# ibrahimhroob/SPS

Hardware: AMD Instinct MI355X
Metric: scans/sec @100k pts, 0.1 m voxel (higher is better)
Workload: dtype f32; 1 GPU; BASELINE config 2: single ~100k-pt LiDAR-like scan + variant-B submap, 0.1 m voxel, CustomMinkUNet14 fp32, 1 scan per step per GPU (4 distinct scans cycled); scan_points=100824, rows=153557, streams_per_gpu=8, compact_arenas=True

## Files before the change

### sps_amd/csrc/grid_kernels.inc.h

```cpp

typedef unsigned int u32x2 __attribute__((ext_vector_type(2)));
constexpr int SCAN_BLOCK = 1024;

struct BHash {
  uint64_t *keys;
  unsigned long long *mask;
  int *first;
  int *rank;
  uint32_t *occ;
  uint32_t hmask;
  uint32_t hshift;
};

constexpr uint32_t BH_X = 0x9E3779B1u, BH_Y = 0x85EBCA77u, BH_Z = 0xC2B2AE3Du, BH_T = 0x27D4EB2Fu;
__device__ inline uint32_t bhash32(uint64_t key) {
  return (uint32_t)(key & 0x3FFFF) * BH_X + (uint32_t)((key >> 18) & 0x3FFFF) * BH_Y + (uint32_t)((key >> 36) & 0x3FFFF) * BH_Z +
         (uint32_t)(key >> 54) * BH_T;
}

__device__ inline int bhash_insert(const BHash &h, uint64_t key) {
  uint32_t s = bhash32(key) >> h.hshift;
  while (true) {
    unsigned long long prev = atomicCAS(reinterpret_cast<unsigned long long *>(&h.keys[s]),
                                        (unsigned long long)KEY_EMPTY, (unsigned long long)key);
    if (prev == KEY_EMPTY) atomicOr(&h.occ[s >> 5], 1u << (s & 31));
    if (prev == KEY_EMPTY || prev == key) return (int)s;
    s = (s + 1) & h.hmask;
  }
}
__device__ inline int bhash_find_from(const BHash &h, uint64_t key, uint32_t s) {
  while (true) {
    if (!((h.occ[s >> 5] >> (s & 31)) & 1u)) return -1;
    if (h.keys[s] == key) return (int)s;
    s = (s + 1) & h.hmask;
  }
}
__device__ inline int bhash_find(const BHash &h, uint64_t key) {
  uint32_t s = bhash32(key) >> h.hshift;
  while (true) {
    if (!((h.occ[s >> 5] >> (s & 31)) & 1u)) return -1;
    if (h.keys[s] == key) return (int)s;
    s = (s + 1) & h.hmask;
  }
}

__device__ inline uint64_t bkey_pack(uint32_t b, uint32_t tt, uint32_t bx, uint32_t by, uint32_t bz) {
  return ((uint64_t)b << 59) | ((uint64_t)tt << 54) | ((uint64_t)bz << 36) | ((uint64_t)by << 18) | (uint64_t)bx;
}

constexpr int NLV = SPS_NUM_LEVELS;

__device__ inline int wave_run_insert(const BHash &h, uint64_t key, bool ok, uint32_t olo, uint32_t ohi, int src) {
  const int lane = threadIdx.x & 63;
  const uint32_t klo = (uint32_t)key, khi = (uint32_t)(key >> 32);
  const uint32_t plo = __shfl_up(klo, 1, 64), phi = __shfl_up(khi, 1, 64);
  const int pok = __shfl_up((int)ok, 1, 64);
  const bool head = !(lane > 0 && ok && pok && plo == klo && phi == khi);
  const unsigned long long heads = __ballot(head);
  const unsigned long long le = heads & (lane == 63 ? ~0ull : ((2ull << lane) - 1ull));
  const int rid = __popcll(le);
  const int head_lane = 63 - __clzll((long long)le);
  if (!ok) {
    olo = 0u;
    ohi = 0u;
  }
#pragma unroll
  for (int o = 1; o < 64; o <<= 1) {
    const uint32_t vlo = __shfl_down(olo, o, 64), vhi = __shfl_down(ohi, o, 64);
    const int r2 = __shfl_down(rid, o, 64);
    if (lane + o < 64 && r2 == rid) {
      olo |= vlo;
      ohi |= vhi;
    }
  }
  int slot = -1;
  if (head && ok) {
    if constexpr (SPS_ABLATE_FE & 1) {
      slot = (int)(bhash32(key) >> h.hshift);
    } else {
      slot = bhash_insert(h, key);
      atomicOr(&h.mask[slot], ((unsigned long long)ohi << 32) | olo);
      atomicMin(&h.first[slot], src);
    }
  }
  return __shfl(slot, head_lane, 64);
}

__global__ __launch_bounds__(256) void k_points_to_blocks(const float *__restrict__ coords, int64_t ld, int n, float vs,
                                                           float t_base, BHash h, int *__restrict__ sslot,
                                                           unsigned char *__restrict__ sbit, int *err,
                                                           uint4 *__restrict__ zero_region, int zero_vec4,
                                                           double *__restrict__ metrics_zero, int metrics_n,
                                                           const int *__restrict__ n_dev) {
  if (n_dev) n = min(n, *n_dev);
  const int p = blockIdx.x * blockDim.x + threadIdx.x;
  if (p < metrics_n) metrics_zero[p] = 0.0;
  for (int i = p; i < zero_vec4; i += gridDim.x * blockDim.x) zero_region[i] = make_uint4(0u, 0u, 0u, 0u);
  bool ok = false;
  uint64_t key = KEY_EMPTY;
  int bit = 0;
  if (p < n) {
    const float *c = coords + (size_t)p * ld;
    const float fb = floorf(__fdiv_rn(c[0], 1.0f));
    const float fx = floorf(__fdiv_rn(c[1], vs));
    const float fy = floorf(__fdiv_rn(c[2], vs));
    const float fz = floorf(__fdiv_rn(c[3], vs));
    const float ft = floorf(__fdiv_rn(c[4], 1.0f)) - t_base;
    ok = fb >= 0.f && fb <= (float)SPS_BATCH_MAX && ft >= (float)SPS_T_MIN && ft <= (float)SPS_T_MAX &&
         fx >= (float)SPS_COORD_MIN && fx <= (float)SPS_COORD_MAX && fy >= (float)SPS_COORD_MIN &&
         fy <= (float)SPS_COORD_MAX && fz >= (float)SPS_COORD_MIN && fz <= (float)SPS_COORD_MAX;
    if (ok) {
      const uint32_t ux = (uint32_t)((int)fx + XBIAS), uy = (uint32_t)((int)fy + XBIAS), uz = (uint32_t)((int)fz + XBIAS);
      key = bkey_pack((uint32_t)(int)fb, (uint32_t)((int)ft + TBIAS), ux >> 2, uy >> 2, uz >> 2);
      bit = (int)(((uz & 3) << 4) | ((uy & 3) << 2) | (ux & 3));
    } else {
      atomicOr(err, 1);
    }
  }
  const int slot = wave_run_insert(h, key, ok, bit < 32 ? (1u << bit) : 0u, bit >= 32 ? (1u << (bit - 32)) : 0u, p);
  if (p < n) {
    sslot[p] = ok ? slot : -1;
    sbit[p] = (unsigned char)bit;
  }
}

struct PyramidArgs {
  BHash h[NLV];
  int *sslot[NLV];
  const unsigned char *sbit0;
  int *bslot[NLV];
  uint64_t *bkey[NLV];
  unsigned long long *bmask[NLV];
  int *bbase[NLV];
  uint4 *bmb[NLV];
  int *bparent[NLV];
  int *bchild[NLV];
  int *badj[NLV];
  int *vblock[NLV];
  unsigned char *vbit[NLV];
  int *counts;
  unsigned long long *agg;
  int agg_stride;
  uint32_t gen;
  const int *n_dev;
  int capl[NLV], bcapl[NLV];
  int *err;
};

constexpr int ABORT = 15;

__device__ inline int block_reduce_sum(int v, int *lds) {
  const int lane = threadIdx.x & 63, wave = threadIdx.x >> 6;
  for (int o = 32; o > 0; o >>= 1) v += __shfl_down(v, o, 64);
  if (lane == 0) lds[wave] = v;
  __syncthreads();
  int tot = 0;
  const int nw = blockDim.x >> 6;
  for (int i = 0; i < nw; ++i) tot += lds[i];
  __syncthreads();
  return tot;
}

constexpr int TICKET = 16, TOCC = 24, N_COUNTERS = 32;

__device__ inline unsigned long long agg_pack(uint32_t gen, int t0, int t1) {
  return ((unsigned long long)gen << 32) | ((unsigned long long)(uint32_t)t1 << 13) | (unsigned long long)(uint32_t)t0;
}
constexpr int SCAN_SPIN_MAX = 1 << 22;
__device__ inline int2 scan_lookback(const unsigned long long *agg, int id, uint32_t gen, int *lds, int *err) {
  if constexpr (SPS_ABLATE_FE & 2) return make_int2(0, 0);
  int p0 = 0, p1 = 0;
  for (int i = threadIdx.x; i < id; i += SCAN_BLOCK) {
    unsigned long long v = __hip_atomic_load(agg + i, __ATOMIC_RELAXED, __HIP_MEMORY_SCOPE_AGENT);
    for (int spin = 0; (uint32_t)(v >> 32) != gen; ++spin) {
      if (spin == SCAN_SPIN_MAX) {
        atomicOr(err, 16);
        v = 0ull;
        break;
      }
      __builtin_amdgcn_s_sleep(1);
      v = __hip_atomic_load(agg + i, __ATOMIC_RELAXED, __HIP_MEMORY_SCOPE_AGENT);
    }
    p0 += (int)(v & 0x1FFFull);
    p1 += (int)((v >> 13) & 0x7FFFFull);
  }
  const int b0 = block_reduce_sum(p0, lds);
  const int b1 = block_reduce_sum(p1, lds);
  return make_int2(b0, b1);
}
__device__ inline int2 block_exclusive_scan2(int v0, int v1, int2 *wave_off, int2 &tot) {
  const int lane = threadIdx.x & 63, wave = threadIdx.x >> 6;
  int i0 = v0, i1 = v1;
  for (int o = 1; o < 64; o <<= 1) {
    const int t0 = __shfl_up(i0, o, 64), t1 = __shfl_up(i1, o, 64);
    if (lane >= o) {
      i0 += t0;
      i1 += t1;
    }
  }
  if (lane == 63) wave_off[wave] = make_int2(i0, i1);
  __syncthreads();
  int o0 = 0, o1 = 0, s0 = 0, s1 = 0;
  for (int i = 0; i < SCAN_BLOCK / 64; ++i) {
    const int2 w = wave_off[i];
    if (i < wave) o0 += w.x, o1 += w.y;
    s0 += w.x, s1 += w.y;
  }
  __syncthreads();
  tot = make_int2(s0, s1);
  return make_int2(o0 + i0 - v0, o1 + i1 - v1);
}

#if defined(SPS_FE_TRACE)
__device__ unsigned long long g_fe_trace[8 * 4096];
#define FE_STAMP(kernel, k) do { if (threadIdx.x == 0) g_fe_trace[8 * ((kernel) * 1024 + blockIdx.x) + (k)] = wall_clock64(); } while (0)
#else
#define FE_STAMP(kernel, k) do { } while (0)
#endif
struct Ranked {
  int flag, slot, rank, base;
  unsigned long long mask;
  uint64_t key;
  int wg_rank0, wg_blocks;
};
template <int ITEMS>
__device__ inline bool rank_pass(const PyramidArgs &a, int l, int n, Ranked &o, int *lds, int2 *wave_off, int *sh_id) {
  FE_STAMP(l != 0, 0);
  if (threadIdx.x == 0) *sh_id = atomicAdd(&a.counts[TICKET + l], 1);
  __syncthreads();
  const int id = *sh_id;
  FE_STAMP(l != 0, 1);
  constexpr int PER_WG = SCAN_BLOCK * ITEMS;
  const int nwg = (n + PER_WG - 1) / PER_WG;
  if (id >= nwg) return false;
  const int p0 = id * PER_WG + (int)threadIdx.x * ITEMS;
  int s[ITEMS], cnt[ITEMS];
  unsigned long long m[ITEMS];
  int flags = 0, nf = 0, nv = 0;
  if (ITEMS == 4 && p0 + 3 < n) {
    const int4 v = *reinterpret_cast<const int4 *>(a.sslot[l] + p0);
    s[0] = v.x, s[1 % ITEMS] = v.y, s[2 % ITEMS] = v.z, s[3 % ITEMS] = v.w;
  } else {
#pragma unroll
    for (int i = 0; i < ITEMS; ++i) s[i] = p0 + i < n ? a.sslot[l][p0 + i] : -1;
  }
  int first[ITEMS];
  uint64_t key[ITEMS];
#pragma unroll
  for (int i = 0; i < ITEMS; ++i) {
    const int si = max(s[i], 0);
    first[i] = a.h[l].first[si];
    m[i] = a.h[l].mask[si];
    key[i] = a.h[l].keys[si];
  }
#pragma unroll
  for (int i = 0; i < ITEMS; ++i) {
    cnt[i] = 0;
    if (s[i] >= 0 && first[i] == p0 + i) {
      flags |= 1 << i;
      cnt[i] = __popcll(m[i]);
      ++nf, nv += cnt[i];
    }
  }
  int2 tot;
  const int2 loc = block_exclusive_scan2(nf, nv, wave_off, tot);
  unsigned long long *agg = a.agg + (size_t)l * a.agg_stride;
  if (threadIdx.x == 0) __hip_atomic_store(agg + id, agg_pack(a.gen, tot.x, tot.y), __ATOMIC_RELAXED, __HIP_MEMORY_SCOPE_AGENT);
  FE_STAMP(l != 0, 2);
  const int2 base = scan_lookback(agg, id, a.gen, lds, a.err);
  FE_STAMP(l != 0, 3);
  int r = base.x + loc.x, vb = base.y + loc.y;
  o.flag = 0;
  o.wg_rank0 = base.x, o.wg_blocks = tot.x;
#pragma unroll
  for (int i = 0; i < ITEMS; ++i) {
    if (((flags >> i) & 1) && r < a.bcapl[l]) {
      a.h[l].rank[s[i]] = r;
      a.bslot[l][r] = s[i];
      a.bkey[l][r] = key[i];
      a.bmask[l][r] = m[i];
      a.bbase[l][r] = vb;
      a.bmb[l][r] = make_uint4((uint32_t)m[i], (uint32_t)(m[i] >> 32), (uint32_t)vb, 0u);
      int4 *ch = reinterpret_cast<int4 *>(a.bchild[l] + (size_t)r * 8);
      ch[0] = make_int4(-1, -1, -1, -1);
      ch[1] = make_int4(-1, -1, -1, -1);
      if (ITEMS == 1) o.flag = 1, o.slot = s[i], o.rank = r, o.base = vb, o.mask = m[i], o.key = key[i];
    }
    if ((flags >> i) & 1) ++r, vb += cnt[i];
  }
  if (id == nwg - 1 && threadIdx.x == 0) {
    const int nb = base.x + tot.x, nvx = base.y + tot.y;
    a.counts[8 + l] = min(nb, a.bcapl[l]);
    a.counts[l] = nvx;
    if (nb > a.bcapl[l] || nvx > a.capl[l]) {
      atomicOr(&a.counts[ABORT], 1);
      atomicOr(a.err, 2);
    }
  }
  return true;
}

__global__ __launch_bounds__(SCAN_BLOCK) void k_rank_points(PyramidArgs a, int n0) {
  __shared__ int lds[SCAN_BLOCK / 64];
  __shared__ int2 wave_off[SCAN_BLOCK / 64];
  __shared__ int sh_id;
  __shared__ uint64_t sh_key[SCAN_BLOCK];
  __shared__ unsigned long long sh_mask[SCAN_BLOCK];
  const int n = a.n_dev ? min(n0, *a.n_dev) : n0;
  Ranked k;
  if (!rank_pass<1>(a, 0, n, k, lds, wave_off, &sh_id)) return;
  FE_STAMP(0, 4);
  uint32_t tb = 0u;
  if (k.flag) {
    const uint64_t key = k.key;
    sh_key[k.rank - k.wg_rank0] = key;
    sh_mask[k.rank - k.wg_rank0] = k.mask;
    tb = 1u << (uint32_t)((key >> 54) & 0x1F);
  }
  for (int o = 32; o > 0; o >>= 1) tb |= __shfl_xor(tb, o, 64);
  if ((threadIdx.x & 63) == 0) lds[threadIdx.x >> 6] = (int)tb;
  __syncthreads();
  if (threadIdx.x == 0) {
    for (int i = 1; i < SCAN_BLOCK / 64; ++i) tb |= (uint32_t)lds[i];
    uint32_t *tocc = reinterpret_cast<uint32_t *>(a.counts) + TOCC;
    if ((__hip_atomic_load(tocc, __ATOMIC_RELAXED, __HIP_MEMORY_SCOPE_AGENT) & tb) != tb) atomicOr(tocc, tb);
  }
  const int nb = min(k.wg_blocks, a.bcapl[0] - k.wg_rank0);
  const int lane = threadIdx.x & 63, wave = threadIdx.x >> 6;
  FE_STAMP(0, 5);
  const int l = 1 + (wave & 3);
  for (int j0 = (wave >> 2) * 64; j0 < nb; j0 += 256) {
    const int j = j0 + lane;
    const bool ok = j < nb;
    uint64_t pkey = KEY_EMPTY;
    unsigned long long pm = 0;
    if (ok) {
      const uint64_t key = sh_key[j];
      const uint32_t bx = (uint32_t)(key & 0x3FFFF), by = (uint32_t)((key >> 18) & 0x3FFFF), bz = (uint32_t)((key >> 36) & 0x3FFFF);
      const uint64_t bt = key & (0x3FFull << 54);
      pkey = bt | ((uint64_t)(bz >> l) << 36) | ((uint64_t)(by >> l) << 18) | (uint64_t)(bx >> l);
      if (l == 1) {
        const unsigned long long m = sh_mask[j];
        const uint32_t ox = bx & 1, oy = by & 1, oz = bz & 1;
#pragma unroll
        for (int kk = 0; kk < 2; ++kk)
#pragma unroll
          for (int jj = 0; jj < 2; ++jj)
#pragma unroll
            for (int i = 0; i < 2; ++i)
              if (m & (0x0000000000330033ull << (2 * i + 8 * jj + 32 * kk)))
                pm |= 1ull << ((2 * oz + kk) * 16 + (2 * oy + jj) * 4 + (2 * ox + i));
      } else {
        const uint32_t px = (bx >> (l - 2)) & 3, py = (by >> (l - 2)) & 3, pz = (bz >> (l - 2)) & 3;
        pm = 1ull << ((pz << 4) | (py << 2) | px);
      }
    }
    const int r = k.wg_rank0 + j;
    int sl = 0;
    if constexpr (!(SPS_ABLATE_FE & 4))
      sl = wave_run_insert(a.h[l], pkey, ok, (uint32_t)pm, (uint32_t)(pm >> 32), r);
    if (ok) a.sslot[l][r] = sl;
  }
#if defined(SPS_FE_TRACE)
  __syncthreads();
  FE_STAMP(0, 6);
#endif
}

constexpr int RANK_ITEMS = 1;
__global__ __launch_bounds__(SCAN_BLOCK) void k_rank_blocks_rows(PyramidArgs a, int gsb, int n0, int *__restrict__ inv) {
  __shared__ int lds[SCAN_BLOCK / 64];
  __shared__ int2 wave_off[SCAN_BLOCK / 64];
  __shared__ int sh_id;
  if ((int)blockIdx.x < 4 * gsb) {
    const int nblk = a.counts[8];
    if (((int)blockIdx.x % gsb) * (SCAN_BLOCK * RANK_ITEMS) >= nblk) return;
    Ranked k;
    rank_pass<RANK_ITEMS>(a, 1 + (int)blockIdx.x / gsb, nblk, k, lds, wave_off, &sh_id);
    FE_STAMP(1, 4);
    return;
  }
  if (a.counts[ABORT]) return;
  FE_STAMP(1, 0);
  const int n = a.n_dev ? min(n0, *a.n_dev) : n0;
  const int p = ((int)blockIdx.x - 4 * gsb) * SCAN_BLOCK + (int)threadIdx.x;
  if (p >= n) return;
  const int s = a.sslot[0][p];
  int row = -1;
  if (s >= 0) {
    const BHash &h = a.h[0];
    const int r = h.rank[s];
    const int bit = a.sbit0[p];
    row = a.bbase[0][r] + __popcll(h.mask[s] & ((1ull << bit) - 1ull));
    a.vblock[0][row] = r;
    a.vbit[0][row] = (unsigned char)bit;
  }
  inv[p] = row;
  FE_STAMP(1, 6);
}

__device__ inline void link_levels(const PyramidArgs &a, int l, int bx, int nbx) {
  const int n = a.counts[8 + l];
  for (int r = bx * 256 + (int)threadIdx.x; r < n; r += nbx * 256) {
    const uint64_t key = a.bkey[l][r];
    const uint32_t bx = (uint32_t)(key & 0x3FFFF), by = (uint32_t)((key >> 18) & 0x3FFFF),
                   bz = (uint32_t)((key >> 36) & 0x3FFFF);
    const uint64_t bt = key & (0x3FFull << 54);
    const uint64_t pkey = bt | ((uint64_t)(bz >> 1) << 36) | ((uint64_t)(by >> 1) << 18) | (uint64_t)(bx >> 1);
    const int ps = bhash_find(a.h[l + 1], pkey);
    const int pr = a.h[l + 1].rank[ps];
    a.bparent[l][r] = pr;
    a.bchild[l + 1][(size_t)pr * 8 + ((bx & 1) | ((by & 1) << 1) | ((bz & 1) << 2))] = r;
    if (l == 0) {
      const unsigned long long m = a.bmask[0][r];
      int sj[NLV], brj[NLV], basej[NLV];
      unsigned long long pmj[NLV];
#pragma unroll
      for (int j = 1; j < NLV; ++j) sj[j] = a.sslot[j][r];
#pragma unroll
      for (int j = 1; j < NLV; ++j) {
        brj[j] = a.h[j].rank[sj[j]];
        pmj[j] = a.h[j].mask[sj[j]];
      }
#pragma unroll
      for (int j = 1; j < NLV; ++j) basej[j] = a.bbase[j][brj[j]];
#pragma unroll
      for (int j = 1; j < NLV; ++j) {
        const int br = brj[j];
        const unsigned long long pmask = pmj[j];
        const int base = basej[j];
        if (j == 1) {
          const uint32_t ox = bx & 1, oy = by & 1, oz = bz & 1;
#pragma unroll
          for (int k = 0; k < 2; ++k)
#pragma unroll
            for (int jj = 0; jj < 2; ++jj)
#pragma unroll
              for (int i = 0; i < 2; ++i)
                if (m & (0x0000000000330033ull << (2 * i + 8 * jj + 32 * k))) {
                  const int bit = (int)((2 * oz + k) * 16 + (2 * oy + jj) * 4 + (2 * ox + i));
                  const int row = base + __popcll(pmask & ((1ull << bit) - 1ull));
                  a.vblock[1][row] = br;
                  a.vbit[1][row] = (unsigned char)bit;
                }
        } else {
          const uint32_t px = (bx >> (j - 2)) & 3, py = (by >> (j - 2)) & 3, pz = (bz >> (j - 2)) & 3;
          const int bit = (int)((pz << 4) | (py << 2) | px);
          const int row = base + __popcll(pmask & ((1ull << bit) - 1ull));
          a.vblock[j][row] = br;
          a.vbit[j][row] = (unsigned char)bit;
        }
      }
    }
  }
}

constexpr int LINK_PER = 3;
#if defined(SPS_FE_TRACE)
__device__ unsigned long long g_link_trace[2 * 16384];
struct LinkStamp {
  __device__ LinkStamp() { if (threadIdx.x == 0 && blockIdx.x < 16384) g_link_trace[2 * blockIdx.x] = wall_clock64(); }
  __device__ ~LinkStamp() { if (threadIdx.x == 0 && blockIdx.x < 16384) g_link_trace[2 * blockIdx.x + 1] = wall_clock64(); }
};
#endif
__global__ __launch_bounds__(256) void k_link_adj(PyramidArgs a, int gb, int c1, int c2, int c3, int c4, int c5) {
  if (a.counts[ABORT]) return;
#if defined(SPS_FE_TRACE)
  LinkStamp stamp;
#endif
  if ((int)blockIdx.x < 4 * gb) {
    link_levels(a, (int)blockIdx.x / gb, (int)blockIdx.x % gb, gb);
    return;
  }
  const int bx = (int)blockIdx.x - 4 * gb;
  const int idx = bx < c1 ? 0 : bx < c2 ? 1 : bx < c3 ? 2 : bx < c4 ? 3 : 4;
  const int level = NLV - 1 - idx;
  const int lo = idx == 0 ? 0 : idx == 1 ? c1 : idx == 2 ? c2 : idx == 3 ? c3 : c4;
  const int hi = idx == 0 ? c1 : idx == 1 ? c2 : idx == 2 ? c3 : idx == 3 ? c4 : c5;
  const int total = a.counts[8 + level] * 27;
  const int lim = 1 << (16 - level);
  const BHash h = a.h[level];
  const uint32_t tocc = reinterpret_cast<const uint32_t *>(a.counts)[TOCC];
  const uint64_t *__restrict__ bkey = a.bkey[level];
  int *__restrict__ badj = a.badj[level];
  const __amdgpu_buffer_rsrc_t rsOcc = __builtin_amdgcn_make_buffer_rsrc((void *)h.occ, 0, (int)0xFFFFFFFEu, 0x00020000);
  const __amdgpu_buffer_rsrc_t rsKeys = __builtin_amdgcn_make_buffer_rsrc((void *)h.keys, 0, (int)0xFFFFFFFEu, 0x00020000);
  const __amdgpu_buffer_rsrc_t rsRank = __builtin_amdgcn_make_buffer_rsrc((void *)h.rank, 0, (int)0xFFFFFFFEu, 0x00020000);
  for (int i = (bx - lo) * 256 + (int)threadIdx.x; i < total; i += (hi - lo) * 256) {
    const int r = i / 27, g = i - r * 27;
    const int dy = g % 3 - 1, dz = (g / 3) % 3 - 1, dt = g / 9 - 1;
    const uint64_t key = bkey[r];
    const int kx = (int)(key & 0x3FFFF), ky = (int)((key >> 18) & 0x3FFFF) + dy, kz = (int)((key >> 36) & 0x3FFFF) + dz,
              tt = (int)((key >> 54) & 0x1F) + dt;
    const bool gok = ky >= 0 && ky < lim && kz >= 0 && kz < lim && tt >= 0 && tt < 32 && ((tocc >> tt) & 1u);
    const uint64_t gkey = key + ((uint64_t)(int64_t)dy << 18) + ((uint64_t)(int64_t)dz << 36) + ((uint64_t)(int64_t)dt << 54);
    const uint32_t ghash = bhash32(key) + (uint32_t)dy * BH_Y + (uint32_t)dz * BH_Z + (uint32_t)dt * BH_T;
    uint64_t nk[LINK_PER];
    uint32_t sl[LINK_PER];
    int res[LINK_PER];
    bool probe[LINK_PER];
#pragma unroll
    for (int j = 0; j < LINK_PER; ++j) {
      const int dx = j - 1;
      const bool self = dx == 0 && g == 13;
      res[j] = self ? r : -1;
      probe[j] = !(SPS_ABLATE_FE & 8) && gok && !self && kx + dx >= 0 && kx + dx < lim;
      nk[j] = gkey + (uint64_t)(int64_t)dx;
      sl[j] = (ghash + (uint32_t)dx * BH_X) >> h.hshift;
    }
    uint32_t ow[LINK_PER];
#pragma unroll
    for (int j = 0; j < LINK_PER; ++j) ow[j] = __builtin_amdgcn_raw_buffer_load_b32(rsOcc, probe[j] ? (sl[j] >> 5) * 4u : 0xFFFFFFFFu, 0, 0);
    uint64_t k1[LINK_PER];
#pragma unroll
    for (int j = 0; j < LINK_PER; ++j) {
      probe[j] = probe[j] && ((ow[j] >> (sl[j] & 31)) & 1u);
      const u32x2 kv = __builtin_amdgcn_raw_buffer_load_b64(rsKeys, probe[j] ? sl[j] * 8u : 0xFFFFFFFFu, 0, 0);
      k1[j] = ((uint64_t)kv.y << 32) | kv.x;
    }
    bool hit[LINK_PER];
    int rk[LINK_PER];
#pragma unroll
    for (int j = 0; j < LINK_PER; ++j) {
      hit[j] = probe[j] && k1[j] == nk[j];
      rk[j] = (int)__builtin_amdgcn_raw_buffer_load_b32(rsRank, hit[j] ? sl[j] * 4u : 0xFFFFFFFFu, 0, 0);
    }
#pragma unroll
    for (int j = 0; j < LINK_PER; ++j) {
      if (hit[j]) {
        res[j] = rk[j];
      } else if (probe[j]) {
        const int s2 = bhash_find_from(h, nk[j], (sl[j] + 1) & h.hmask);
        if (s2 >= 0) res[j] = h.rank[s2];
      }
    }
    int *__restrict__ o = badj + (size_t)r * 81 + g * 3;
    if constexpr (SPS_ABLATE_FE & 16) {
      if (g == 13) o[1] = res[1];
    } else {
#pragma unroll
      for (int j = 0; j < LINK_PER; ++j) o[j] = res[j];
    }
  }
}

__device__ inline void bhash_cleanup(const PyramidArgs &a, int l, int bx, int nbx) {
  const int n = a.counts[8 + l];
  const BHash h = a.h[l];
  if (a.counts[ABORT]) {
    const uint32_t slots = h.hmask + 1u;
    for (uint32_t s = (uint32_t)bx * 256u + threadIdx.x; s < slots; s += (uint32_t)nbx * 256u) {
      h.keys[s] = KEY_EMPTY;
      h.mask[s] = 0ull;
      h.first[s] = 0x7F7F7F7F;
      if ((s & 31u) == 0u) h.occ[s >> 5] = 0u;
    }
    return;
  }
  for (int r = bx * 256 + (int)threadIdx.x; r < n; r += nbx * 256) {
    const int s = a.bslot[l][r];
    h.keys[s] = KEY_EMPTY;
    h.mask[s] = 0ull;
    h.first[s] = 0x7F7F7F7F;
    h.occ[s >> 5] = 0u;
  }
}
```

### sps_amd/csrc/sps_hip.hip

```cpp
#include <hip/hip_runtime.h>

#include <cmath>
#include <cstdarg>
#include <cstdint>
#include <cstdio>
#include <algorithm>
#include <array>
#include <cstdlib>
#include <cstring>
#include <map>
#include <memory>
#include <string>
#include <vector>

#include "../../include/sps_hip.h"

#if !defined(SPS_DIAG)
#undef SPS_ABLATE_A
#undef SPS_ABLATE_B
#undef SPS_ABLATE_HALF_B
#undef SPS_ABLATE_SKIP_B
#undef SPS_ABLATE_MFMA
#undef SPS_ABLATE_LOOP
#undef SPS_ABLATE_STAGE
// ... 1047 lines not shown
  if (rc != SPS_OK) return rc;
  rc = sps_ctx_set_weights(c, h);
  delete h;
  return rc;
}

struct ForwardOpts {
  bool head = false;
  const float *feats = nullptr;
  float t_base = 0.f;
  int64_t ldo = 1;
  int act = 0;
  double *metrics_out = nullptr;
  float eps = 0.f;
  int n_batches = 0;
  const int *n_dev = nullptr;
  bool front_only = false;
};

static int forward_impl(sps_ctx *c, const float *coords, int64_t ld, int64_t n, float vs, float *scores,
                        const ForwardOpts &fo, void *stream);

int sps_forward(sps_ctx *c, const float *coords, int64_t ld, int64_t n, float vs, float *scores, void *stream) {
  if (c && c->have_weights && c->net->out_channels != 1)
    return fail(SPS_ERR_INVALID, "the loaded weights have a %d-channel head: use sps_forward_head", c->net->out_channels);
  return forward_impl(c, coords, ld, n, vs, scores, ForwardOpts{}, stream);
}

int sps_forward_n(sps_ctx *c, const float *coords, int64_t ld, int64_t n_max, const int32_t *n_dev, float vs, float *scores,
                  void *stream) {
  if (c && c->have_weights && c->net->out_channels != 1)
    return fail(SPS_ERR_INVALID, "the loaded weights have a %d-channel head: use sps_forward_head", c->net->out_channels);
  if (!n_dev) return fail(SPS_ERR_INVALID, "n_dev is null");
  ForwardOpts fo;
  fo.n_dev = n_dev;
  return forward_impl(c, coords, ld, n_max, vs, scores, fo, stream);
}

int sps_forward_head(sps_ctx *c, const float *coords, int64_t ld, int64_t n, float vs, const float *feats, float t_base,
                     float *out, int64_t ldo, int activation, void *stream) {
  if (c && c->have_weights && ldo < c->net->out_channels) return fail(SPS_ERR_INVALID, "ldo is smaller than out_channels");
  if (activation != 0 && activation != 1) return fail(SPS_ERR_INVALID, "activation must be 0 (none) or 1 (sigmoid)");
  if (!(t_base == floorf(t_base)) || fabsf(t_base) > 16777216.f) return fail(SPS_ERR_INVALID, "t_base must be an integer");
  ForwardOpts fo;
  fo.head = true;
  fo.feats = feats;
  fo.t_base = t_base;
  fo.ldo = ldo;
  fo.act = activation;
  return forward_impl(c, coords, ld, n, vs, out, fo, stream);
}

int sps_forward_metrics(sps_ctx *c, const float *batch, int64_t ld, int64_t n, float vs, float eps, int n_batches,
                        float *scores, double *out_dev, void *stream) {
  if (c && c->have_weights && c->net->out_channels != 1)
    return fail(SPS_ERR_INVALID, "the loaded weights have a %d-channel head: use sps_forward_head", c->net->out_channels);
  if (!out_dev) return fail(SPS_ERR_INVALID, "null argument");
  if (n_batches < 1 || n_batches > 31) return fail(SPS_ERR_INVALID, "n_batches must be in [1,31]");
  if (ld < 6) return fail(SPS_ERR_INVALID, "rows must carry (b,x,y,z,t,label): ld >= 6");
  if (n == 0) {
    HIP_TRY(hipSetDevice(c ? c->device : 0));
    HIP_TRY(hipMemsetAsync(out_dev, 0, (size_t)n_batches * 8 * sizeof(double), (hipStream_t)stream));
  }
  ForwardOpts fo;
  fo.metrics_out = out_dev;
  fo.eps = eps;
  fo.n_batches = n_batches;
  return forward_impl(c, batch, ld, n, vs, scores, fo, stream);
}

int sps_forward_metrics_n(sps_ctx *c, const float *batch, int64_t ld, int64_t n_max, const int32_t *n_dev, float vs, float eps,
                          int n_batches, float *scores, double *out_dev, void *stream) {
  if (c && c->have_weights && c->net->out_channels != 1)
    return fail(SPS_ERR_INVALID, "the loaded weights have a %d-channel head: use sps_forward_head", c->net->out_channels);
  if (!out_dev || !n_dev) return fail(SPS_ERR_INVALID, "null argument");
  if (n_batches < 1 || n_batches > 31) return fail(SPS_ERR_INVALID, "n_batches must be in [1,31]");
  if (ld < 6) return fail(SPS_ERR_INVALID, "rows must carry (b,x,y,z,t,label): ld >= 6");
  if (n_max == 0) {
    HIP_TRY(hipSetDevice(c ? c->device : 0));
    HIP_TRY(hipMemsetAsync(out_dev, 0, (size_t)n_batches * 8 * sizeof(double), (hipStream_t)stream));
  }
  ForwardOpts fo;
  fo.metrics_out = out_dev;
  fo.eps = eps;
  fo.n_batches = n_batches;
  fo.n_dev = n_dev;
  return forward_impl(c, batch, ld, n_max, vs, scores, fo, stream);
}

#if defined(SPS_FE_TRACE)
static int g_maps_geom[8], g_link_geom[8];
#endif
static int forward_impl(sps_ctx *c, const float *coords, int64_t ld, int64_t n, float vs, float *scores,
                        const ForwardOpts &fo, void *stream) {
  if (!c) return fail(SPS_ERR_INVALID, "ctx is null");
  if (!c->have_weights) return fail(SPS_ERR_NOWEIGHTS, "sps_weights_load has not been called");
  if (n < 0 || ld < 5 || (n > 0 && (!coords || !scores))) return fail(SPS_ERR_INVALID, "bad arguments");
  if (!(vs > 0.f)) return fail(SPS_ERR_INVALID, "voxel_size must be > 0");
  if (n > SPS_MAX_POINTS) return fail(SPS_ERR_INVALID, "too many points (limit %d)", SPS_MAX_POINTS);
  HIP_TRY(hipSetDevice(c->device));
  hipStream_t st = (hipStream_t)stream;
  if (n > c->cap || c->regrow) {
    int rc = reserve(c, n);
    if (rc != SPS_OK) return rc;
  }
  static const int diag_skip = [] { const char *e = diag_env("SPS_DIAG_SKIP"); return e ? atoi(e) : 0; }();
  static const int no_merge = [] { const char *e = diag_env("SPS_NO_MERGE"); return e ? atoi(e) : 0; }();
  const bool skip_front = (diag_skip & 1) && c->last_n == n && c->diag_have_state;
  const bool skip_convs = (diag_skip & 2) != 0;
  c->last_n = n;
  ++c->fwd_gen;
  const int64_t cap = c->cap;
  c->prof_n = 0;
  prof_mark(c, "begin", st);
  Level &L0 = c->lv[0];
  PyramidArgs pa = pyramid_args(c);
  pa.n_dev = fo.n_dev;
  if (!skip_front) {
  if (c->tables_dirty) {
    HIP_TRY(hipMemsetAsync(c->hash_keys_all, 0xFF, (size_t)c->hash_slots * sizeof(uint64_t), st));
    HIP_TRY(hipMemsetAsync(c->hash_mask_all, 0, (size_t)c->hash_slots * sizeof(unsigned long long), st));
    HIP_TRY(hipMemsetAsync(c->hash_first_all, 0x7F, (size_t)c->hash_slots * sizeof(int), st));
    HIP_TRY(hipMemsetAsync(c->hash_occ_all, 0, (size_t)(c->hash_slots / 32) * sizeof(uint32_t), st));
  }
  if (c->tables_dirty) HIP_TRY(hipMemsetAsync(c->zero_region, 0, c->zero_bytes, st));
  c->tables_dirty = true;
  if (n == 0) {
    HIP_TRY(hipMemsetAsync(c->zero_region, 0, c->zero_bytes, st));
    c->tables_dirty = false;
    return SPS_OK;
  }
  prof_mark(c, "reset", st);

  const unsigned gp = (unsigned)((n + 255) / 256);
  const unsigned gs0 = (unsigned)((n + SCAN_BLOCK - 1) / SCAN_BLOCK);
  const unsigned gsb = (unsigned)((cap + SCAN_BLOCK * RANK_ITEMS - 1) / (SCAN_BLOCK * RANK_ITEMS));
  hipLaunchKernelGGL(k_points_to_blocks, dim3(gp), dim3(256), 0, st, coords, ld, (int)n, vs, fo.t_base, L0.h, L0.sslot, L0.sbit,
                     c->err, reinterpret_cast<uint4 *>(c->zero_region), (int)(c->zero_bytes / 16), fo.metrics_out,
                     fo.metrics_out ? fo.n_batches * 8 : 0, fo.n_dev);
  hipLaunchKernelGGL(k_rank_points, dim3(gs0), dim3(SCAN_BLOCK), 0, st, pa, (int)n);
  hipLaunchKernelGGL(k_rank_blocks_rows, dim3(4 * gsb + gs0), dim3(SCAN_BLOCK), 0, st, pa, (int)gsb, (int)n, L0.inv);
  const int gb = grid_for(cap >> 2, 256, 256);
  if (fo.feats) {
    HIP_TRY(hipMemsetAsync(c->vacc, 0, (size_t)n * sizeof(long long), st));
    HIP_TRY(hipMemsetAsync(c->vcnt, 0, (size_t)n * sizeof(int), st));
    hipLaunchKernelGGL(k_voxel_feat_accum, dim3(gp), dim3(256), 0, st, fo.feats, L0.inv, (int)n, c->vacc, c->vcnt, fo.n_dev);
    hipLaunchKernelGGL(k_voxel_feat_mean, dim3((unsigned)grid_for(n, 256, 2048)), dim3(256), 0, st, c->counts, c->vacc,
                       c->vcnt, c->vfeat);
  }
  c->last_kernel = "k_points_to_blocks+k_rank_points+k_rank_blocks_rows";
  prof_mark(c, "voxelize", st);
  {
    int co[NLV + 1] = {0};
    for (int i = 0; i < NLV; ++i) co[i + 1] = co[i] + grid_for(((cap >> 3) >> (2 * (NLV - 1 - i))) * 27, 256, 2048);
#if defined(SPS_FE_TRACE)
    g_link_geom[0] = gb;
    for (int l = 0; l <= NLV; ++l) g_link_geom[1 + l] = co[l];
#endif
    if (no_merge & 2) {
      hipLaunchKernelGGL(k_link_adj, dim3(4 * gb), dim3(256), 0, st, pa, gb, co[1], co[2], co[3], co[4], co[5]);
      hipLaunchKernelGGL(k_link_adj, dim3(co[NLV]), dim3(256), 0, st, pa, 0, co[1], co[2], co[3], co[4], co[5]);
    } else {
      hipLaunchKernelGGL(k_link_adj, dim3(4 * gb + co[NLV]), dim3(256), 0, st, pa, gb, co[1], co[2], co[3], co[4], co[5]);
    }
  }
  c->last_kernel = "k_link_adj";
  prof_mark(c, "pyramid", st);
  MapsArgs ma{};
  int off = 0;
  for (int l = 0; l < NLV; ++l) {
    const Level &L = c->lv[l];
    ma.L[l] = L.view();
    ma.nbr3[l] = L.nbr3;
    ma.tm3[l] = L.tm3;
    ma.down[l] = L.down;
    ma.parent_row[l] = L.inv;
    ma.tmdown[l] = L.tmdown;
    ma.chunk_off[l] = off;
    off += grid_for(cap >> l, 256, 1024);
  }
  ma.chunk_off[NLV] = off;
  ma.counts = c->counts;
  for (int l = 0; l < PX_LEVELS; ++l)
    if (((px_levels() >> l) & 1) && !fo.front_only) ma.rb_e[l] = c->lv[l].rb_e, ma.rb_k[l] = c->lv[l].rb_k, ma.rb_cnt[l] = c->lv[l].rb_cnt;
  for (int l = 0; l < NLV; ++l) ma.ldn[l] = c->capl[l];
#if defined(SPS_FE_TRACE)
  g_maps_geom[0] = off;
  for (int l = 0; l <= NLV; ++l) g_maps_geom[1 + l] = ma.chunk_off[l];
#endif
  if (no_merge & 4) {
    hipLaunchKernelGGL(k_maps, dim3(off * 3), dim3(256), 0, st, ma, off, off * 3);
    hipLaunchKernelGGL(k_maps, dim3(ma.chunk_off[NLV - 1]), dim3(256), 0, st, ma, off, 0);
  } else {
    hipLaunchKernelGGL(k_maps, dim3(off * 3 + ma.chunk_off[NLV - 1]), dim3(256), 0, st, ma, off, off * 3);
  }
  c->diag_have_state = true;
  }
  c->last_kernel = "k_maps";
  prof_mark(c, "maps", st);
  if (fo.front_only) {
    HIP_TRY(hipGetLastError());
    return SPS_OK;
  }
  Level *lv = c->lv;
  c->cur_vfeat = fo.feats ? c->vfeat : nullptr;
  const bool fuse_final = !fo.head;
  const ConvCall calls[] = {
      {"conv0p1s1", nullptr, 1, c->cat8 + 8, 16, Map{c->nbr5, c->tm5}, 0, nullptr, 0, 1},
      {"conv1p1s2", c->cat8 + 8, 16, c->x1, 8, Map{lv[1].down, lv[1].tmdown}, 1, nullptr, 0, 1},
      {"block1.0.conv1", c->x1, 8, c->b1t, 8, Map{lv[1].nbr3, lv[1].tm3}, 1, nullptr, 0, 1},
      {"block1.0.conv2", c->b1t, 8, c->cat7 + 16, 24, Map{lv[1].nbr3, lv[1].tm3}, 1, c->x1, 8, 1},
      {"conv2p2s2", c->cat7 + 16, 24, c->x2, 8, Map{lv[2].down, lv[2].tmdown}, 2, nullptr, 0, 1},
      {"block2.0.conv1", c->x2, 8, c->b2t, 16, Map{lv[2].nbr3, lv[2].tm3}, 2, nullptr, 0, 1},
      {"block2.0.conv2", c->b2t, 16, c->cat6 + 32, 48, Map{lv[2].nbr3, lv[2].tm3}, 2, nullptr, 0, 1, c->x2, 8},
      {"conv3p4s2", c->cat6 + 32, 48, c->x3, 16, Map{lv[3].down, lv[3].tmdown}, 3, nullptr, 0, 1},
      {"block3.0.conv1", c->x3, 16, c->b3t, 32, Map{lv[3].nbr3, lv[3].tm3}, 3, nullptr, 0, 1},
      {"block3.0.conv2", c->b3t, 32, c->cat5 + 64, 96, Map{lv[3].nbr3, lv[3].tm3}, 3, nullptr, 0, 1, c->x3, 16},
      {"conv4p8s2", c->cat5 + 64, 96, c->x4, 32, Map{lv[4].down, lv[4].tmdown}, 4, nullptr, 0, 1},
      {"block4.0.conv1", c->x4, 32, c->b4t, 64, Map{lv[4].nbr3, lv[4].tm3}, 4, nullptr, 0, 1},
      {"block4.0.conv2", c->b4t, 64, c->b4o, 64, Map{lv[4].nbr3, lv[4].tm3}, 4, nullptr, 0, 1, c->x4, 32, false,
       (FUSE_UP & 1) ? "convtr4p16s2" : nullptr, c->cat5, 96},
      {"convtr4p16s2", c->b4o, 64, c->cat5, 96, Map{lv[4].down, lv[4].tmdown}, 3, nullptr, 0, 1},
      {"block5.0.conv1", c->cat5, 96, c->b5t, 64, Map{lv[3].nbr3, lv[3].tm3}, 3, nullptr, 0, 1},
      {"block5.0.conv2", c->b5t, 64, c->b5o, 64, Map{lv[3].nbr3, lv[3].tm3}, 3, nullptr, 0, 1, c->cat5, 96, false,
       (FUSE_UP & 2) ? "convtr5p8s2" : nullptr, c->cat6, 48},
      {"convtr5p8s2", c->b5o, 64, c->cat6, 48, Map{lv[3].down, lv[3].tmdown}, 2, nullptr, 0, 1},
      {"block6.0.conv1", c->cat6, 48, c->b6t, 32, Map{lv[2].nbr3, lv[2].tm3}, 2, nullptr, 0, 1},
      {"block6.0.conv2", c->b6t, 32, c->b6o, 32, Map{lv[2].nbr3, lv[2].tm3}, 2, nullptr, 0, 1, c->cat6, 48, false,
       (FUSE_UP & 4) ? "convtr6p4s2" : nullptr, c->cat7, 24},
      {"convtr6p4s2", c->b6o, 32, c->cat7, 24, Map{lv[2].down, lv[2].tmdown}, 1, nullptr, 0, 1},
      {"block7.0.conv1", c->cat7, 24, c->b7t, 16, Map{lv[1].nbr3, lv[1].tm3}, 1, nullptr, 0, 1},
      {"block7.0.conv2", c->b7t, 16, c->b7o, 16, Map{lv[1].nbr3, lv[1].tm3}, 1, nullptr, 0, 1, c->cat7, 24, false,
       (FUSE_UP & 8) ? "convtr7p2s2" : nullptr, c->cat8, 16},
      {"convtr7p2s2", c->b7o, 16, c->cat8, 16, Map{lv[1].down, lv[1].tmdown}, 0, nullptr, 0, 1},
      {"block8.0.conv1", c->cat8, 16, c->b8t, 8, Map{lv[0].nbr3, lv[0].tm3}, 0, nullptr, 0, 1},
      {"block8.0.conv2", c->b8t, 8, c->b8o, 8, Map{lv[0].nbr3, lv[0].tm3}, 0, nullptr, 0, 1, c->cat8, 16, fuse_final},
  };
  const char *fused_up = nullptr;
  static const char *const fused_stage[][2] = {{"block4.0.conv2", "block4.0.conv2+convtr4p16s2"},
                                               {"block5.0.conv2", "block5.0.conv2+convtr5p8s2"},
                                               {"block6.0.conv2", "block6.0.conv2+convtr6p4s2"},
                                               {"block7.0.conv2", "block7.0.conv2+convtr7p2s2"}};
  static const int skip_class = [] { const char *e = diag_env("SPS_DIAG_SKIP_CLASS"); return e ? atoi(e) : 0; }();
  for (const ConvCall &cc : calls) {
    if (skip_convs) break;
    if (skip_class) {
      const bool tr = std::strncmp(cc.name, "convtr", 6) == 0, c0 = std::strcmp(cc.name, "conv0p1s1") == 0;
      const bool blk = std::strncmp(cc.name, "block", 5) == 0, strided = !tr && !c0 && !blk;
      const int cls = blk ? (cc.level_out >= 2 ? 1 : 2) : strided ? 4 : tr ? 8 : 16;
      if (skip_class & cls) continue;
    }
    if (fused_up && std::strcmp(cc.name, fused_up) == 0) {
      fused_up = nullptr;
      continue;
    }
    int rc = run_conv(c, cc, st);
    if (rc != SPS_OK) return rc;
    const char *stage = cc.name;
    if (cc.up) {
      fused_up = cc.up;
      for (const auto &fs : fused_stage)
        if (std::strcmp(cc.name, fs[0]) == 0) stage = fs[1];
    }
    prof_mark(c, stage, st);
  }
  c->cur_vfeat = nullptr;
  const int gs = (int)((n + 255) / 256), gbc = grid_for(cap >> 2, 256, 256);
  if (fo.head) {
    const NetSpec &s = *c->net;
    const ConvSpec &fs = s.convs[s.find_conv("final")];
    hipLaunchKernelGGL(k_slice_head, dim3((unsigned)gs), dim3(256), 0, st, c->b8o, 8, L0.inv, (int)n,
                       c->blob + fs.w_off, c->blob + s.bias_off, s.out_channels, fo.act, scores, fo.ldo, c->counts + 15,
                       fo.n_dev);
    c->last_kernel = "k_slice_head";
    prof_mark(c, "slice_head", st);
    if (!skip_front) hipLaunchKernelGGL(k_bhash_cleanup, dim3(gbc * NLV), dim3(256), 0, st, pa, gbc);
  } else if (skip_front || (no_merge & 8)) {
    hipLaunchKernelGGL(k_slice_sigmoid, dim3((unsigned)gs), dim3(256), 0, st, c->logits, L0.inv, (int)n, scores, c->counts + 15);
    if (!skip_front) hipLaunchKernelGGL(k_bhash_cleanup, dim3(gbc * NLV), dim3(256), 0, st, pa, gbc);
    if (fo.metrics_out) {
      HIP_TRY(hipMemsetAsync(fo.metrics_out, 0, (size_t)fo.n_batches * 8 * sizeof(double), st));
      hipLaunchKernelGGL(k_metrics, dim3((unsigned)grid_for(n, 1024, 128)), dim3(256), 0, st, scores, (int)n,
                         MetricsArgs{coords, ld, fo.eps, fo.n_batches, fo.metrics_out});
    }
  } else {
    const MetricsArgs mt{coords, ld, fo.eps, fo.n_batches, fo.metrics_out};
    const int gst = fo.metrics_out ? grid_for(n, 1024, 256) : gs;
    hipLaunchKernelGGL(k_tail, dim3((unsigned)(gst + gbc * NLV)), dim3(256), 0, st, c->logits, L0.inv, (int)n, scores, gst,
                       pa, gbc, mt);
  }
  c->last_kernel = fo.head ? "k_bhash_cleanup" : "k_tail";
  prof_mark(c, "tail", st);
  HIP_TRY(hipGetLastError());
  c->tables_dirty = false;
  return SPS_OK;
}

#include "train_host.inc.h"

static void train_destroy(sps_ctx *c) {
  if (!c->train) return;
  train_free(c->train);
  delete c->train;
  c->train = nullptr;
}

int sps_profile_enable(sps_ctx *c, int on) {
// ... 699 lines not shown
```

Before: 4132 scans/s.

## Restructure link/rank front-end kernels: early counter loads, 9-wide adjacency probes, prefetched keys

Changes several front-end pyramid kernels to hide latency. k_link_adj now gives each thread 9 neighbor entries instead of 3, which cuts the thread count and repeated key/hash work. It also batches the occupancy, key and rank buffer loads and handles collisions with a vectorised second probe before falling back to a serial walk. The abort and count checks move from early-exit global loads to buffer loads issued alongside the data loads, and the next key is prefetched each iteration. link_levels uses a direct hash-slot probe for the parent lookup and reuses the rank of the already-known level-1 slot for level 0. The scan lookback issues its first aggregate load before the block scan. The price is more register pressure from the 9-wide arrays and more complex control flow.

```diff
diff --git a/sps_amd/csrc/grid_kernels.inc.h b/sps_amd/csrc/grid_kernels.inc.h
--- a/sps_amd/csrc/grid_kernels.inc.h
+++ b/sps_amd/csrc/grid_kernels.inc.h
@@ -167,11 +167,15 @@
   return ((unsigned long long)gen << 32) | ((unsigned long long)(uint32_t)t1 << 13) | (unsigned long long)(uint32_t)t0;
 }
 constexpr int SCAN_SPIN_MAX = 1 << 22;
-__device__ inline int2 scan_lookback(const unsigned long long *agg, int id, uint32_t gen, int *lds, int *err) {
+__device__ inline unsigned long long scan_peek(const unsigned long long *agg, int id) {
+  return (int)threadIdx.x < id ? __hip_atomic_load(agg + threadIdx.x, __ATOMIC_RELAXED, __HIP_MEMORY_SCOPE_AGENT) : 0ull;
+}
+__device__ inline int2 scan_lookback(const unsigned long long *agg, int id, uint32_t gen, int *lds, int *err,
+                                     unsigned long long peek) {
   if constexpr (SPS_ABLATE_FE & 2) return make_int2(0, 0);
   int p0 = 0, p1 = 0;
   for (int i = threadIdx.x; i < id; i += SCAN_BLOCK) {
-    unsigned long long v = __hip_atomic_load(agg + i, __ATOMIC_RELAXED, __HIP_MEMORY_SCOPE_AGENT);
+    unsigned long long v = i == (int)threadIdx.x ? peek : __hip_atomic_load(agg + i, __ATOMIC_RELAXED, __HIP_MEMORY_SCOPE_AGENT);
     for (int spin = 0; (uint32_t)(v >> 32) != gen; ++spin) {
       if (spin == SCAN_SPIN_MAX) {
         atomicOr(err, 16);
@@ -253,6 +257,8 @@
     m[i] = a.h[l].mask[si];
     key[i] = a.h[l].keys[si];
   }
+  unsigned long long *agg = a.agg + (size_t)l * a.agg_stride;
+  const unsigned long long peek = scan_peek(agg, id);
 #pragma unroll
   for (int i = 0; i < ITEMS; ++i) {
     cnt[i] = 0;
@@ -264,10 +270,9 @@
   }
   int2 tot;
   const int2 loc = block_exclusive_scan2(nf, nv, wave_off, tot);
-  unsigned long long *agg = a.agg + (size_t)l * a.agg_stride;
   if (threadIdx.x == 0) __hip_atomic_store(agg + id, agg_pack(a.gen, tot.x, tot.y), __ATOMIC_RELAXED, __HIP_MEMORY_SCOPE_AGENT);
   FE_STAMP(l != 0, 2);
-  const int2 base = scan_lookback(agg, id, a.gen, lds, a.err);
+  const int2 base = scan_lookback(agg, id, a.gen, lds, a.err, peek);
   FE_STAMP(l != 0, 3);
   int r = base.x + loc.x, vb = base.y + loc.y;
   o.flag = 0;
@@ -380,17 +385,20 @@
     FE_STAMP(1, 4);
     return;
   }
-  if (a.counts[ABORT]) return;
   FE_STAMP(1, 0);
+  const int p = ((int)blockIdx.x - 4 * gsb) * SCAN_BLOCK + (int)threadIdx.x;
+  if (p >= n0) return;
+  const int v_abort = (int)__builtin_amdgcn_raw_buffer_load_b32(
+      __builtin_amdgcn_make_buffer_rsrc((void *)a.counts, 0, N_COUNTERS * 4, 0x00020000), ABORT * 4u, 0, 0);
+  const int s = a.sslot[0][p];
+  const int bit = a.sbit0[p];
   const int n = a.n_dev ? min(n0, *a.n_dev) : n0;
-  const int p = ((int)blockIdx.x - 4 * gsb) * SCAN_BLOCK + (int)threadIdx.x;
+  if (v_abort != 0) return;
   if (p >= n) return;
-  const int s = a.sslot[0][p];
   int row = -1;
   if (s >= 0) {
     const BHash &h = a.h[0];
     const int r = h.rank[s];
-    const int bit = a.sbit0[p];
     row = a.bbase[0][r] + __popcll(h.mask[s] & ((1ull << bit) - 1ull));
     a.vblock[0][row] = r;
     a.vbit[0][row] = (unsigned char)bit;
@@ -399,24 +407,47 @@
   FE_STAMP(1, 6);
 }
 
+__device__ inline __amdgpu_buffer_rsrc_t counters_rsrc(const PyramidArgs &a) {
+  return __builtin_amdgcn_make_buffer_rsrc((void *)a.counts, 0, N_COUNTERS * 4, 0x00020000);
+}
+__device__ inline int counter_load(__amdgpu_buffer_rsrc_t rs, int k) {
+  return (int)__builtin_amdgcn_raw_buffer_load_b32(rs, (uint32_t)k * 4u, 0, 0);
+}
+#define COUNTERS_USED_FROM_HERE(x, y) asm volatile("" : "+v"(x), "+v"(y))
+
 __device__ inline void link_levels(const PyramidArgs &a, int l, int bx, int nbx) {
-  const int n = a.counts[8 + l];
-  for (int r = bx * 256 + (int)threadIdx.x; r < n; r += nbx * 256) {
-    const uint64_t key = a.bkey[l][r];
+  const __amdgpu_buffer_rsrc_t rsCnt = counters_rsrc(a);
+  int v_abort = counter_load(rsCnt, ABORT), n = counter_load(rsCnt, 8 + l);
+  const int bcap = a.bcapl[l];
+  const __amdgpu_buffer_rsrc_t rsKey = __builtin_amdgcn_make_buffer_rsrc((void *)a.bkey[l], 0, bcap * 8, 0x00020000);
+  const BHash hp = a.h[l + 1];
+  u32x2 kv = __builtin_amdgcn_raw_buffer_load_b64(rsKey, (uint32_t)(bx * 256 + (int)threadIdx.x) * 8u, 0, 0);
+  for (int r = bx * 256 + (int)threadIdx.x; r < bcap; r += nbx * 256) {
+    int sj[NLV];
+    unsigned long long m = 0ull;
+    if (l == 0) {
+      m = a.bmask[0][r];
+#pragma unroll
+      for (int j = 1; j < NLV; ++j) sj[j] = a.sslot[j][r];
+    }
+    COUNTERS_USED_FROM_HERE(v_abort, n);
+    if (v_abort != 0 || r >= n) break;
+    const uint64_t key = ((uint64_t)kv.y << 32) | kv.x;
     const uint32_t bx = (uint32_t)(key & 0x3FFFF), by = (uint32_t)((key >> 18) & 0x3FFFF),
                    bz = (uint32_t)((key >> 36) & 0x3FFFF);
-    const uint64_t bt = key & (0x3FFull << 54);
-    const uint64_t pkey = bt | ((uint64_t)(bz >> 1) << 36) | ((uint64_t)(by >> 1) << 18) | (uint64_t)(bx >> 1);
-    const int ps = bhash_find(a.h[l + 1], pkey);
-    const int pr = a.h[l + 1].rank[ps];
-    a.bparent[l][r] = pr;
-    a.bchild[l + 1][(size_t)pr * 8 + ((bx & 1) | ((by & 1) << 1) | ((bz & 1) << 2))] = r;
-    if (l == 0) {
-      const unsigned long long m = a.bmask[0][r];
-      int sj[NLV], brj[NLV], basej[NLV];
+    const int oct = (int)((bx & 1) | ((by & 1) << 1) | ((bz & 1) << 2));
+    if (l != 0) {
+      const uint64_t bt = key & (0x3FFull << 54);
+      const uint64_t pkey = bt | ((uint64_t)(bz >> 1) << 36) | ((uint64_t)(by >> 1) << 18) | (uint64_t)(bx >> 1);
+      const uint32_t s = bhash32(pkey) >> hp.hshift;
+      const uint64_t k1 = hp.keys[s];
+      int pr = hp.rank[s];
+      if (k1 != pkey) pr = hp.rank[bhash_find_from(hp, pkey, (s + 1) & hp.hmask)];
+      a.bparent[l][r] = pr;
+      a.bchild[l + 1][(size_t)pr * 8 + oct] = r;
+    } else {
+      int brj[NLV], basej[NLV];
       unsigned long long pmj[NLV];
-#pragma unroll
-      for (int j = 1; j < NLV; ++j) sj[j] = a.sslot[j][r];
 #pragma unroll
       for (int j = 1; j < NLV; ++j) {
         brj[j] = a.h[j].rank[sj[j]];
@@ -424,6 +455,8 @@
       }
 #pragma unroll
       for (int j = 1; j < NLV; ++j) basej[j] = a.bbase[j][brj[j]];
+      a.bparent[0][r] = brj[1];
+      a.bchild[1][(size_t)brj[1] * 8 + oct] = r;
 #pragma unroll
       for (int j = 1; j < NLV; ++j) {
         const int br = brj[j];
@@ -452,10 +485,16 @@
         }
       }
     }
-  }
-}
-
-constexpr int LINK_PER = 3;
+    kv = __builtin_amdgcn_raw_buffer_load_b64(rsKey, (uint32_t)(r + nbx * 256) * 8u, 0, 0);
+  }
+}
+
+#ifndef SPS_LINK_PER
+#define SPS_LINK_PER 9
+#endif
+constexpr int LINK_PER = SPS_LINK_PER;
+constexpr int LINK_GROUPS = 81 / LINK_PER;
+static_assert(LINK_PER == 9 || LINK_PER == 3, "a thread owns whole dx runs of the 81 entries");
 #if defined(SPS_FE_TRACE)
 __device__ unsigned long long g_link_trace[2 * 16384];
 struct LinkStamp {
@@ -464,7 +503,6 @@
 };
 #endif
 __global__ __launch_bounds__(256) void k_link_adj(PyramidArgs a, int gb, int c1, int c2, int c3, int c4, int c5) {
-  if (a.counts[ABORT]) return;
 #if defined(SPS_FE_TRACE)
   LinkStamp stamp;
 #endif
@@ -477,70 +515,112 @@
   const int level = NLV - 1 - idx;
   const int lo = idx == 0 ? 0 : idx == 1 ? c1 : idx == 2 ? c2 : idx == 3 ? c3 : c4;
   const int hi = idx == 0 ? c1 : idx == 1 ? c2 : idx == 2 ? c3 : idx == 3 ? c4 : c5;
-  const int total = a.counts[8 + level] * 27;
   const int lim = 1 << (16 - level);
   const BHash h = a.h[level];
-  const uint32_t tocc = reinterpret_cast<const uint32_t *>(a.counts)[TOCC];
-  const uint64_t *__restrict__ bkey = a.bkey[level];
   int *__restrict__ badj = a.badj[level];
+  const int bcap = a.bcapl[level];
+  const __amdgpu_buffer_rsrc_t rsCnt = counters_rsrc(a);
+  const __amdgpu_buffer_rsrc_t rsBkey = __builtin_amdgcn_make_buffer_rsrc((void *)a.bkey[level], 0, bcap * 8, 0x00020000);
   const __amdgpu_buffer_rsrc_t rsOcc = __builtin_amdgcn_make_buffer_rsrc((void *)h.occ, 0, (int)0xFFFFFFFEu, 0x00020000);
   const __amdgpu_buffer_rsrc_t rsKeys = __builtin_amdgcn_make_buffer_rsrc((void *)h.keys, 0, (int)0xFFFFFFFEu, 0x00020000);
   const __amdgpu_buffer_rsrc_t rsRank = __builtin_amdgcn_make_buffer_rsrc((void *)h.rank, 0, (int)0xFFFFFFFEu, 0x00020000);
-  for (int i = (bx - lo) * 256 + (int)threadIdx.x; i < total; i += (hi - lo) * 256) {
-    const int r = i / 27, g = i - r * 27;
-    const int dy = g % 3 - 1, dz = (g / 3) % 3 - 1, dt = g / 9 - 1;
-    const uint64_t key = bkey[r];
-    const int kx = (int)(key & 0x3FFFF), ky = (int)((key >> 18) & 0x3FFFF) + dy, kz = (int)((key >> 36) & 0x3FFFF) + dz,
+  constexpr uint32_t OOR = 0xFFFFFFFFu;
+  int v_abort = counter_load(rsCnt, ABORT);
+  int nblk = counter_load(rsCnt, 8 + level);
+  const uint32_t tocc = (uint32_t)counter_load(rsCnt, TOCC);
+  const int i0 = (bx - lo) * 256 + (int)threadIdx.x, istep = (hi - lo) * 256;
+  u32x2 kv0 = __builtin_amdgcn_raw_buffer_load_b64(rsBkey, (uint32_t)(i0 / LINK_GROUPS) * 8u, 0, 0);
+  for (int i = i0; i < bcap * LINK_GROUPS; i += istep) {
+    const int r = i / LINK_GROUPS, g = i - r * LINK_GROUPS;
+    COUNTERS_USED_FROM_HERE(v_abort, nblk);
+    if (v_abort != 0 || r >= nblk) break;
+    const uint64_t key = ((uint64_t)kv0.y << 32) | kv0.x;
+    const int dy0 = LINK_PER == 9 ? 0 : g % 3 - 1;
+    const int dz = LINK_PER == 9 ? g % 3 - 1 : (g / 3) % 3 - 1;
+    const int dt = LINK_PER == 9 ? g / 3 - 1 : g / 9 - 1;
+    const int e0 = g * LINK_PER;
+    const int kx = (int)(key & 0x3FFFF), ky = (int)((key >> 18) & 0x3FFFF) + dy0, kz = (int)((key >> 36) & 0x3FFFF) + dz,
               tt = (int)((key >> 54) & 0x1F) + dt;
-    const bool gok = ky >= 0 && ky < lim && kz >= 0 && kz < lim && tt >= 0 && tt < 32 && ((tocc >> tt) & 1u);
-    const uint64_t gkey = key + ((uint64_t)(int64_t)dy << 18) + ((uint64_t)(int64_t)dz << 36) + ((uint64_t)(int64_t)dt << 54);
-    const uint32_t ghash = bhash32(key) + (uint32_t)dy * BH_Y + (uint32_t)dz * BH_Z + (uint32_t)dt * BH_T;
-    uint64_t nk[LINK_PER];
+    const bool gok = kz >= 0 && kz < lim && tt >= 0 && tt < 32 && ((tocc >> tt) & 1u);
+    const uint64_t gkey = key + ((uint64_t)(int64_t)dy0 << 18) + ((uint64_t)(int64_t)dz << 36) + ((uint64_t)(int64_t)dt << 54);
+    const uint32_t ghash = bhash32(key) + (uint32_t)dy0 * BH_Y + (uint32_t)dz * BH_Z + (uint32_t)dt * BH_T;
+#define LINK_KD(j) ((uint64_t)(int64_t)((j) % 3 - 1) + ((uint64_t)(int64_t)(LINK_PER == 9 ? (j) / 3 - 1 : 0) << 18))
     uint32_t sl[LINK_PER];
+    bool probe[LINK_PER];
+#pragma unroll
+    for (int j = 0; j < LINK_PER; ++j) {
+      const int dx = j % 3 - 1, ddy = LINK_PER == 9 ? j / 3 - 1 : 0;
+      const bool self = e0 + j == 40;
+      probe[j] = !(SPS_ABLATE_FE & 8) && gok && !self && kx + dx >= 0 && kx + dx < lim && ky + ddy >= 0 &&
+                 ky + ddy < lim;
+      sl[j] = (ghash + (uint32_t)dx * BH_X + (uint32_t)ddy * BH_Y) >> h.hshift;
+    }
+    uint32_t ow[LINK_PER];
+#pragma unroll
+    for (int j = 0; j < LINK_PER; ++j) ow[j] = __builtin_amdgcn_raw_buffer_load_b32(rsOcc, probe[j] ? (sl[j] >> 5) * 4u : OOR, 0, 0);
+    uint64_t k1[LINK_PER];
     int res[LINK_PER];
-    bool probe[LINK_PER];
-#pragma unroll
-    for (int j = 0; j < LINK_PER; ++j) {
-      const int dx = j - 1;
-      const bool self = dx == 0 && g == 13;
-      res[j] = self ? r : -1;
-      probe[j] = !(SPS_ABLATE_FE & 8) && gok && !self && kx + dx >= 0 && kx + dx < lim;
-      nk[j] = gkey + (uint64_t)(int64_t)dx;
-      sl[j] = (ghash + (uint32_t)dx * BH_X) >> h.hshift;
-    }
-    uint32_t ow[LINK_PER];
-#pragma unroll
-    for (int j = 0; j < LINK_PER; ++j) ow[j] = __builtin_amdgcn_raw_buffer_load_b32(rsOcc, probe[j] ? (sl[j] >> 5) * 4u : 0xFFFFFFFFu, 0, 0);
-    uint64_t k1[LINK_PER];
 #pragma unroll
     for (int j = 0; j < LINK_PER; ++j) {
       probe[j] = probe[j] && ((ow[j] >> (sl[j] & 31)) & 1u);
-      const u32x2 kv = __builtin_amdgcn_raw_buffer_load_b64(rsKeys, probe[j] ? sl[j] * 8u : 0xFFFFFFFFu, 0, 0);
+      const u32x2 kv = __builtin_amdgcn_raw_buffer_load_b64(rsKeys, probe[j] ? sl[j] * 8u : OOR, 0, 0);
       k1[j] = ((uint64_t)kv.y << 32) | kv.x;
-    }
-    bool hit[LINK_PER];
-    int rk[LINK_PER];
+      res[j] = (int)__builtin_amdgcn_raw_buffer_load_b32(rsRank, probe[j] ? sl[j] * 4u : OOR, 0, 0);
+    }
+    uint32_t coll = 0u;
 #pragma unroll
     for (int j = 0; j < LINK_PER; ++j) {
-      hit[j] = probe[j] && k1[j] == nk[j];
-      rk[j] = (int)__builtin_amdgcn_raw_buffer_load_b32(rsRank, hit[j] ? sl[j] * 4u : 0xFFFFFFFFu, 0, 0);
-    }
-#pragma unroll
-    for (int j = 0; j < LINK_PER; ++j) {
-      if (hit[j]) {
-        res[j] = rk[j];
-      } else if (probe[j]) {
-        const int s2 = bhash_find_from(h, nk[j], (sl[j] + 1) & h.hmask);
-        if (s2 >= 0) res[j] = h.rank[s2];
-      }
-    }
-    int *__restrict__ o = badj + (size_t)r * 81 + g * 3;
+      const bool hit = probe[j] && k1[j] - gkey == LINK_KD(j);
+      if (probe[j] && !hit) coll |= 1u << j;
+      res[j] = hit ? res[j] : (e0 + j == 40 ? r : -1);
+    }
+    if (coll != 0u) {
+#pragma unroll
+      for (int j = 0; j < LINK_PER; ++j) {
+        sl[j] = (sl[j] + 1) & h.hmask;
+        ow[j] = __builtin_amdgcn_raw_buffer_load_b32(rsOcc, ((coll >> j) & 1u) ? (sl[j] >> 5) * 4u : OOR, 0, 0);
+      }
+#pragma unroll
+      for (int j = 0; j < LINK_PER; ++j) {
+        probe[j] = ((coll >> j) & 1u) && ((ow[j] >> (sl[j] & 31)) & 1u);
+        const u32x2 kv = __builtin_amdgcn_raw_buffer_load_b64(rsKeys, probe[j] ? sl[j] * 8u : OOR, 0, 0);
+        k1[j] = ((uint64_t)kv.y << 32) | kv.x;
+      }
+      uint32_t walk = 0u;
+      int r2[LINK_PER];
+#pragma unroll
+      for (int j = 0; j < LINK_PER; ++j) {
+        const bool hit = probe[j] && k1[j] - gkey == LINK_KD(j);
+        if (probe[j] && !hit) walk |= 1u << j;
+        probe[j] = hit;
+        r2[j] = (int)__builtin_amdgcn_raw_buffer_load_b32(rsRank, hit ? sl[j] * 4u : OOR, 0, 0);
+      }
+#pragma unroll
+      for (int j = 0; j < LINK_PER; ++j) res[j] = probe[j] ? r2[j] : res[j];
+      while (walk != 0u) {
+        const int j = __ffs((int)walk) - 1;
+        walk &= walk - 1u;
+        uint32_t s = 0u;
+#pragma unroll
+        for (int k = 0; k < LINK_PER; ++k) s = j == k ? sl[k] : s;
+        const uint64_t wkey = gkey + (uint64_t)(int64_t)(j % 3 - 1) + ((uint64_t)(int64_t)(LINK_PER == 9 ? j / 3 - 1 : 0) << 18);
+        const int s3 = bhash_find_from(h, wkey, (s + 1) & h.hmask);
+        if (s3 >= 0) {
+          const int v = h.rank[s3];
+#pragma unroll
+          for (int k = 0; k < LINK_PER; ++k) res[k] = j == k ? v : res[k];
+        }
+      }
+    }
+#undef LINK_KD
+    int *__restrict__ o = badj + (size_t)r * 81 + e0;
     if constexpr (SPS_ABLATE_FE & 16) {
-      if (g == 13) o[1] = res[1];
+      if (e0 <= 40 && 40 < e0 + LINK_PER) o[40 - e0] = r;
     } else {
 #pragma unroll
       for (int j = 0; j < LINK_PER; ++j) o[j] = res[j];
     }
+    kv0 = __builtin_amdgcn_raw_buffer_load_b64(rsBkey, (uint32_t)((i + istep) / LINK_GROUPS) * 8u, 0, 0);
   }
 }
 
diff --git a/sps_amd/csrc/sps_hip.hip b/sps_amd/csrc/sps_hip.hip
--- a/sps_amd/csrc/sps_hip.hip
+++ b/sps_amd/csrc/sps_hip.hip
@@ -1223,7 +1223,7 @@
   prof_mark(c, "voxelize", st);
   {
     int co[NLV + 1] = {0};
-    for (int i = 0; i < NLV; ++i) co[i + 1] = co[i] + grid_for(((cap >> 3) >> (2 * (NLV - 1 - i))) * 27, 256, 2048);
+    for (int i = 0; i < NLV; ++i) co[i + 1] = co[i] + grid_for(((cap >> 3) >> (2 * (NLV - 1 - i))) * LINK_GROUPS, 256, 2048);
 #if defined(SPS_FE_TRACE)
     g_link_geom[0] = gb;
     for (int l = 0; l <= NLV; ++l) g_link_geom[1 + l] = co[l];
```

Result: no change. 4098 scans/s (-0.8%).
